# brudfors/UniRes

Measured on AMD Instinct MI355X. Metric: cg_iters_per_sec, higher is better.
Workload: dtype f32

## Files before the change

include/unires_hip.h:

```cpp
#ifndef UNIRES_HIP_H
#define UNIRES_HIP_H

#include <stdint.h>

#ifdef __cplusplus
extern "C" {
#endif

#define UNIRES_HIP_ABI_VERSION 1
#define UNIRES_MAX_TAPS 32

enum unires_status {
  UNIRES_OK = 0,
  UNIRES_ERR_NULL = 1,
  UNIRES_ERR_DIM = 2,
  UNIRES_ERR_ARG = 3,
  UNIRES_ERR_HIP = 4,
  UNIRES_ERR_ALLOC = 5,
  UNIRES_ERR_UNSUPPORTED = 6
};

enum unires_operator { UNIRES_OP_A = 0, UNIRES_OP_AT = 1, UNIRES_OP_ATA = 2 };

enum unires_regime {
// ... 48 lines not shown

int unires_div_fwd_zero(const float *src3, const int32_t dim[3], const float vx[3], float *dst,
                        void *stream);

int unires_dtd(const float *src, const int32_t dim[3], const float vx[3], float a, float c,
               float *dst, void *stream);


typedef struct unires_repeat {
  int32_t dim_x[3];
  int32_t dim_g[3];
  float M[12];
  int32_t ratio[3];
  int32_t ntaps[3];
  const float *taps[3];
  float scl;
  int32_t dim_thick;
  float tau;
} unires_repeat_t;

typedef struct unires_plan unires_plan_t;

int unires_plan_create(unires_plan_t **plan, const int32_t dim_y[3], const float vx_y[3],
                       int32_t regime, int32_t n_repeats, const unires_repeat_t *repeats,
                       float fov_tol);
int unires_plan_destroy(unires_plan_t *plan);
int unires_plan_set_repeat(unires_plan_t *plan, int32_t n, const unires_repeat_t *repeat);
int unires_plan_set_concurrency(unires_plan_t *plan, int32_t n_concurrent);
int64_t unires_plan_workspace_bytes(const unires_plan_t *plan);
int unires_plan_repeat_info(const unires_plan_t *plan, int32_t n, int32_t info[8]);
int unires_orient_of(const float M[12], int32_t perm[3], int32_t flip[3]);
int unires_plan_time_matvecs(unires_plan_t *plan, int32_t on);
int unires_plan_matvec_time(unires_plan_t *plan, int32_t *launches, double *total_us);

int unires_proj_apply(unires_plan_t *plan, int32_t n, int32_t op, const float *in, float *out,
                      void *stream);

int unires_ata_matvec(unires_plan_t *plan, float rho, float lam, const float *p, float *q,
                      double *dot_dev, void *stream);

int unires_rhs_assemble(unires_plan_t *plan, const float *const *x_ptrs, const float *w_c,
                        const float *z_c, float rho, float lam, float *b, void *stream);

int unires_atx_assemble(unires_plan_t *plan, const float *const *x_ptrs, float *atx,
                        void *stream);

int unires_rhs_from_atx(unires_plan_t *plan, const float *atx, const float *w_c,
                        const float *z_c, float rho, float lam, float *b, void *stream);

int unires_precond_build(unires_plan_t *plan, int32_t precond_mode, float rho, float lam,
                         float *m_out, void *stream);

int unires_precond_apply(unires_plan_t *plan, const float *in, float *out, void *stream);

int unires_cg_solve(unires_plan_t *plan, float rho, float lam, const float *b, float *x,
                    int32_t max_iter, double tol, int32_t stop_mode, int32_t precond_mode,
                    int32_t *iters_out, double *obj_trace, void *stream);

int unires_cg_solve_many(int32_t n, unires_plan_t *const *plans, const float *rho, const float *lam,
                         const float *const *b, float *const *x, int32_t max_iter, double tol,
                         int32_t stop_mode, int32_t precond_mode, int32_t *iters_out,
                         double *obj_trace, void *const *streams);


int unires_zw_update(const float *const *y_ptrs, const float *lam, int32_t n_channels,
                     const int32_t dim[3], const float vx[3], float rho, float alpha, float *z,
// ... 27 lines not shown
```

unires_amd/_lib.py:

```python
import ctypes as C
import os

_HERE = os.path.dirname(os.path.abspath(__file__))
LIB_PATH = os.environ.get('UNIRES_LIB') or os.path.join(_HERE, 'libunires_hip.so')

UNIRES_MAX_TAPS = 32
OP = {'A': 0, 'At': 1, 'AtA': 2}
REGIME_IDENTITY, REGIME_DENOISE, REGIME_SUPERRES = 0, 1, 2
STOP = {'e': 0, 'max_gain': 3, 'max_gain_guarded': 3, 'max_gain_fresh': 1, 'max_gain_recurred': 2}
PRECOND = {'none': 0, 'identity': 0, 'jacobi': 1, 'fft': 2}

c_i32x3 = C.c_int32 * 3
c_f32x3 = C.c_float * 3
c_f32x12 = C.c_float * 12
c_fptrx3 = C.POINTER(C.c_float) * 3


class Repeat(C.Structure):
    _fields_ = [('dim_x', c_i32x3), ('dim_g', c_i32x3), ('M', c_f32x12), ('ratio', c_i32x3),
                ('ntaps', c_i32x3), ('taps', c_fptrx3), ('scl', C.c_float),
                ('dim_thick', C.c_int32), ('tau', C.c_float)]


SIGNATURES = {
    'unires_last_error': (C.c_char_p, []),
    'unires_abi_version': (C.c_int, []),
    'unires_pull3d_affine': (C.c_int, [C.c_void_p, c_i32x3, c_f32x12, C.c_void_p, c_i32x3,
                                       C.c_float, C.c_void_p]),
    'unires_warp_label': (C.c_int, [C.c_void_p, c_i32x3, c_f32x12, C.c_void_p, c_i32x3,
                                    C.c_float, C.c_void_p]),
    'unires_pull3d_nearest': (C.c_int, [C.c_void_p, c_i32x3, c_f32x12, C.c_void_p, c_i32x3,
                                        C.c_float, C.c_void_p]),
    'unires_pull_grad3d_affine': (C.c_int, [C.c_void_p, c_i32x3, c_f32x12, C.c_void_p, c_i32x3,
                                            C.c_float, C.c_void_p]),
    'unires_push3d_affine': (C.c_int, [C.c_void_p, c_i32x3, c_f32x12, C.c_void_p, c_i32x3,
                                       C.c_float, C.c_float, C.c_int, C.c_void_p]),
    'unires_conv_down3d': (C.c_int, [C.c_void_p, c_i32x3, c_fptrx3, c_i32x3, c_i32x3, C.c_void_p,
                                     c_i32x3, C.c_float, C.c_int32, C.c_void_p]),
    'unires_conv_up3d': (C.c_int, [C.c_void_p, c_i32x3, c_fptrx3, c_i32x3, c_i32x3, C.c_void_p,
                                   c_i32x3, C.c_float, C.c_int32, C.c_void_p]),
    'unires_grad_fwd_zero': (C.c_int, [C.c_void_p, c_i32x3, c_f32x3, C.c_void_p, C.c_void_p]),
    'unires_div_fwd_zero': (C.c_int, [C.c_void_p, c_i32x3, c_f32x3, C.c_void_p, C.c_void_p]),
    'unires_dtd': (C.c_int, [C.c_void_p, c_i32x3, c_f32x3, C.c_float, C.c_float, C.c_void_p,
                             C.c_void_p]),
    'unires_plan_create': (C.c_int, [C.POINTER(C.c_void_p), c_i32x3, c_f32x3, C.c_int32,
                                     C.c_int32, C.POINTER(Repeat), C.c_float]),
    'unires_plan_destroy': (C.c_int, [C.c_void_p]),
    'unires_plan_set_repeat': (C.c_int, [C.c_void_p, C.c_int32, C.POINTER(Repeat)]),
    'unires_plan_set_concurrency': (C.c_int, [C.c_void_p, C.c_int32]),
    'unires_plan_workspace_bytes': (C.c_int64, [C.c_void_p]),
    'unires_orient_of': (C.c_int, [c_f32x12, c_i32x3, c_i32x3]),
    'unires_plan_repeat_info': (C.c_int, [C.c_void_p, C.c_int32, C.c_int32 * 8]),
    'unires_plan_time_matvecs': (C.c_int, [C.c_void_p, C.c_int32]),
    'unires_plan_matvec_time': (C.c_int, [C.c_void_p, C.POINTER(C.c_int32), C.POINTER(C.c_double)]),
    'unires_proj_apply': (C.c_int, [C.c_void_p, C.c_int32, C.c_int32, C.c_void_p, C.c_void_p,
                                    C.c_void_p]),
    'unires_ata_matvec': (C.c_int, [C.c_void_p, C.c_float, C.c_float, C.c_void_p, C.c_void_p,
                                    C.c_void_p, C.c_void_p]),
    'unires_rhs_assemble': (C.c_int, [C.c_void_p, C.POINTER(C.c_void_p), C.c_void_p, C.c_void_p,
                                      C.c_float, C.c_float, C.c_void_p, C.c_void_p]),
    'unires_atx_assemble': (C.c_int, [C.c_void_p, C.POINTER(C.c_void_p), C.c_void_p, C.c_void_p]),
    'unires_rhs_from_atx': (C.c_int, [C.c_void_p, C.c_void_p, C.c_void_p, C.c_void_p, C.c_float,
                                      C.c_float, C.c_void_p, C.c_void_p]),
    'unires_precond_build': (C.c_int, [C.c_void_p, C.c_int32, C.c_float, C.c_float, C.c_void_p,
                                       C.c_void_p]),
    'unires_precond_apply': (C.c_int, [C.c_void_p, C.c_void_p, C.c_void_p, C.c_void_p]),
    'unires_cg_solve': (C.c_int, [C.c_void_p, C.c_float, C.c_float, C.c_void_p, C.c_void_p,
                                  C.c_int32, C.c_double, C.c_int32, C.c_int32,
                                  C.POINTER(C.c_int32), C.POINTER(C.c_double), C.c_void_p]),
    'unires_cg_solve_many': (C.c_int, [C.c_int32, C.POINTER(C.c_void_p), C.POINTER(C.c_float),
                                       C.POINTER(C.c_float), C.POINTER(C.c_void_p), C.POINTER(C.c_void_p),
                                       C.c_int32, C.c_double, C.c_int32, C.c_int32, C.POINTER(C.c_int32),
                                       C.POINTER(C.c_double), C.POINTER(C.c_void_p)]),
    'unires_zw_update': (C.c_int, [C.POINTER(C.c_void_p), C.POINTER(C.c_float), C.c_int32, c_i32x3,
                                   c_f32x3, C.c_float, C.c_float, C.c_void_p, C.c_void_p,
                                   C.c_void_p, C.c_void_p]),
    'unires_nll_prior': (C.c_int, [C.POINTER(C.c_void_p), C.POINTER(C.c_float), C.c_int32, c_i32x3,
                                   c_f32x3, C.c_void_p, C.c_void_p]),
    'unires_scaling_sums': (C.c_int, [C.c_void_p, C.c_void_p, c_i32x3, C.c_int32, C.c_void_p,
                                      C.c_void_p]),
    'unires_rigid_sums': (C.c_int, [C.c_void_p, C.c_void_p, C.c_void_p, c_i32x3, C.c_float * 72,
                                    C.c_void_p, C.c_void_p]),
    'unires_clean_fov': (C.c_int, [C.c_void_p, c_i32x3, c_f32x12, c_i32x3, C.c_void_p]),
    'unires_masked_sse': (C.c_int, [C.c_void_p, C.c_void_p, C.c_int64, C.c_void_p, C.c_void_p]),
    'unires_mark_create': (C.c_int, [C.POINTER(C.c_void_p)]),
    'unires_mark_destroy': (C.c_int, [C.c_void_p]),
    'unires_mark_signal': (C.c_int, [C.c_void_p, C.c_uint64, C.c_void_p]),
# ... 45 lines not shown
```

unires_amd/_plan.py:

```python
import ctypes as C

import numpy as np
import torch

from . import _lib
from ._lib import (REGIME_DENOISE, REGIME_IDENTITY, REGIME_SUPERRES, Repeat, check, f3, i3)
from ._ops import FOV_TOL, _ptr, _stream, _vol, on_device
from .spatial import _m12, voxel_size


def proj_matrix(po, method):
    if method == 'super-resolution':
        return torch.linalg.solve(po.mat_y, po.rigid.mm(po.mat_yx)), tuple(po.dim_yx)
    if method == 'denoising':
        return torch.linalg.solve(po.mat_y, po.rigid.mm(po.mat_x)), tuple(po.dim_x)
    raise ValueError('Undefined method')


def regime_of(method, do_proj):
    if method not in ('denoising', 'super-resolution'):
        raise ValueError('Undefined method')
    if not do_proj:
        return REGIME_IDENTITY
    return REGIME_SUPERRES if method == 'super-resolution' else REGIME_DENOISE
# ... 50 lines not shown
    def rhs_buffer(self, like):
        buf = getattr(self, '_rhs_buf', None)
        if buf is None or buf.shape != like.shape or buf.device != like.device:
            buf = torch.empty_like(like)
            self._rhs_buf = buf
        return buf

    def close(self):
        if getattr(self, '_h', None) is not None and self._h:
            try:
                with torch.cuda.device(self.device):
                    self.lib.unires_plan_destroy(self._h)
            except Exception:
                self.lib.unires_plan_destroy(self._h)
            self._h = None

    __del__ = close

    @property
    def workspace_bytes(self):
        return int(self.lib.unires_plan_workspace_bytes(self._h))

    def repeat_info(self, n):
        info = (C.c_int32 * 8)()
        check(self.lib.unires_plan_repeat_info(self._h, int(n), info))
        v = list(info)
        return dict(perm=tuple(v[:3]), flip=tuple((v[3] >> j) & 1 for j in range(3)), pull2=bool(v[4]),
                    splat2_axis=None if v[5] == 0 else v[5] - 2, shift=bool(v[6] & 1), separable=bool(v[7]),
                    fused=bool(v[6] & 2))

    @on_device
    def time_matvecs(self, on=True):
        check(self.lib.unires_plan_time_matvecs(self._h, 2 if on == 2 else (1 if on else 0)))

    @on_device
    def matvec_time(self):
        n, us = C.c_int32(0), C.c_double(0.0)
        check(self.lib.unires_plan_matvec_time(self._h, C.byref(n), C.byref(us)))
        return int(n.value), float(us.value)

    @on_device
    def set_repeat(self, n, po, tau):
        keep = []
        r = _repeat_desc(po, tau, self.method, self.regime, keep)
        check(self.lib.unires_plan_set_repeat(self._h, n, C.byref(r)))

    def set_concurrency(self, n):
        n = max(1, int(n))
        if n != self._concurrency:
            check(self.lib.unires_plan_set_concurrency(self._h, n))
            self._concurrency = n

    def _y(self, t, name):
        v, _ = _vol(t, name)
        if tuple(v.shape) != self.dim_y:
            raise ValueError('unires_amd: %s has shape %s, expected %s'
                             % (name, tuple(v.shape), self.dim_y))
        return v

    @on_device
    def proj_apply(self, n, operator, dat):
        if operator not in _lib.OP:
            raise ValueError('Undefined operator')
        d, lead = _vol(dat)
        out_dim = self.dims_x[n] if operator == 'A' else self.dim_y
        in_dim = self.dims_x[n] if operator == 'At' else self.dim_y
# ... 137 lines not shown
```

unires_amd/csrc/api.hip:

```cpp
#include <math.h>
#include <stdio.h>
#include <stdlib.h>
#include <string.h>

#include <time.h>

#include <functional>
#include <map>
#include <mutex>
#include <new>
#include <string>
#include <vector>

#include "admm.hpp"
#include "aligned.hpp"
#include "cg.hpp"
#include "fftpre.hpp"
#include "fused.hpp"
#include "ops.hpp"
#include "orient.hpp"
#include "pull2.hpp"
#include "shift.hpp"
#include "splat2.hpp"
#include "ata1.hpp"
// ... 268 lines not shown
  int ctab_n = 0, ctab_cap = 0;
  unsigned ctab_step = 1, src_stride = 1;
  float *xytab_dev[2] = {nullptr, nullptr};
  int xytab_cap[2] = {0, 0};
  PullPlan pplan;
  ShiftPlan shift;
  F1Sched f1;
};

struct unires_plan {
  Dim3i dy;
  float vx[3];
  int regime;
  float fov_tol;
  std::vector<Repeat> reps;
  char *ws = nullptr;
  size_t ws_bytes = 0;
  float *r = nullptr, *p = nullptr, *ap = nullptr, *ax = nullptr;
  bool timing = false;
  bool twice = false;
  std::vector<std::pair<hipEvent_t, hipEvent_t>> tev;
  float *gbuf = nullptr;
  float *gbuf2 = nullptr;
  float *xbuf = nullptr;
  float *xperm = nullptr;
  double *part0 = nullptr, *part1 = nullptr;
  CgState *state = nullptr;
  size_t cap_g = 0, cap_x = 0;
  struct CgKey {
    const float *b = nullptr;
    float *x = nullptr;
    float rho = 0.f, lam = 0.f;
    int max_iter = -1, stop = -1, pre = -1;
    double tol = -1.0;
    bool operator==(const CgKey &o) const {
      return b == o.b && x == o.x && rho == o.rho && lam == o.lam && max_iter == o.max_iter &&
             stop == o.stop && pre == o.pre && tol == o.tol;
    }
  } cg_key;
  hipGraphExec_t cg_exec = nullptr;
  CgKey cg_chunk_key;
  hipGraphExec_t cg_start_exec = nullptr, cg_chunk_exec = nullptr;
  unsigned long long *progress = nullptr, *progress_dev = nullptr;
  unsigned cg_gen = 0;
  float *precM = nullptr;
  FftPre fft;
  float prec_rho = 0.f, prec_lam = 0.f;
  int prec_mode = UNIRES_PRECOND_IDENTITY;
  bool prec_ready = false;
  hipEvent_t last_use = nullptr;
  std::vector<hipStream_t> use_streams;
  bool captured_use = false;
  int concurrency = 1;
  int cap_s2 = 0, cap_f1 = 0;
};

static void drop_timing(unires_plan *pl) {
  for (auto &e : pl->tev) (void)hipEventDestroy(e.first), (void)hipEventDestroy(e.second);
  pl->tev.clear();
}

static void mark_use(unires_plan *pl, hipStream_t st) {
  hipStreamCaptureStatus cs = hipStreamCaptureStatusNone;
  if (hipStreamIsCapturing(st, &cs) != hipSuccess) {
    (void)hipGetLastError();
    cs = hipStreamCaptureStatusNone;
  }
  if (cs != hipStreamCaptureStatusNone) {
    pl->captured_use = true;
    return;
  }
  for (hipStream_t s : pl->use_streams)
    if (s == st) return;
  if (pl->use_streams.size() >= 8)
    pl->captured_use = true;
  else
    pl->use_streams.push_back(st);
}
// ... 337 lines not shown
  pl->ax = (float *)(pl->ws + o_ax);
  pl->gbuf = (float *)(pl->ws + o_g);
  pl->xbuf = (float *)(pl->ws + o_x);
  pl->xperm = (float *)(pl->ws + o_xp);
  pl->gbuf2 = need_sep ? (float *)(pl->ws + o_g2) : nullptr;
  pl->part0 = (double *)(pl->ws + o_p0);
  pl->part1 = (double *)(pl->ws + o_p1);
  pl->state = (CgState *)(pl->ws + o_st);
  e = hipMemset(pl->state, 0, sizeof(CgState));
  if (e != hipSuccess) {
    g_err = std::string("hipMemset: ") + hipGetErrorString(e);
    (void)hipFree(pl->ws);
    delete pl;
    return UNIRES_ERR_HIP;
  }
  for (Repeat &R : pl->reps) {
    int rc = UNIRES_OK;
    if (!rc) rc = build_repeat_kernels(pl, R);
    if (rc) {
      for (Repeat &Q : pl->reps) free_sched(Q);
      (void)hipFree(pl->ws);
      delete pl;
      return rc;
    }
  }
  *plan = pl;
  return UNIRES_OK;
}

extern "C" int unires_plan_destroy(unires_plan_t *plan) {
  if (!plan) return UNIRES_OK;
  if (plan->ws) (void)hipFree(plan->ws);
  if (plan->precM) (void)hipFree(plan->precM);
  if (plan->cg_exec) (void)hipGraphExecDestroy(plan->cg_exec);
  if (plan->cg_start_exec) (void)hipGraphExecDestroy(plan->cg_start_exec);
  if (plan->cg_chunk_exec) (void)hipGraphExecDestroy(plan->cg_chunk_exec);
  if (plan->progress) (void)hipHostFree(plan->progress);
  if (plan->last_use) (void)hipEventDestroy(plan->last_use);
  drop_timing(plan);
  fftpre_destroy(plan->fft);
  for (Repeat &R : plan->reps) free_sched(R);
  delete plan;
  return UNIRES_OK;
}

extern "C" int unires_plan_time_matvecs(unires_plan_t *plan, int32_t on) {
  if (!plan) return fail(UNIRES_ERR_NULL, "null argument");
  const bool twice = on == 2;
  if (twice != plan->twice) drop_cg_graph(plan);
  plan->twice = twice;
  plan->timing = on == 1;
  if (!plan->timing) drop_timing(plan);
  return UNIRES_OK;
}

extern "C" int unires_plan_matvec_time(unires_plan_t *plan, int32_t *launches, double *total_us) {
  if (!plan || !launches || !total_us) return fail(UNIRES_ERR_NULL, "null argument");
  *launches = 0, *total_us = 0.0;
  for (auto &e : plan->tev) {
    float ms = 0.f;
    HIP_TRY(hipEventSynchronize(e.second));
    HIP_TRY(hipEventElapsedTime(&ms, e.first, e.second));
    *total_us += 1e3 * (double)ms;
    ++*launches;
  }
  drop_timing(plan);
  return UNIRES_OK;
}

extern "C" int unires_plan_set_repeat(unires_plan_t *plan, int32_t n,
                                      const unires_repeat_t *repeat) {
  if (!plan || !repeat) return fail(UNIRES_ERR_NULL, "null argument");
  if (n < 0 || n >= (int)plan->reps.size()) return fail(UNIRES_ERR_ARG, "repeat index");
  Repeat tmp;
  int rc = fill_repeat(plan, repeat, tmp);
  if (rc) return rc;
  if (plan->regime != UNIRES_REGIME_IDENTITY &&
      (tmp.dim_g.numel() > plan->cap_g || tmp.dim_x.numel() > plan->cap_x))
    return fail(UNIRES_ERR_DIM, "new repeat exceeds the plan's workspace");
  if (plan->regime == UNIRES_REGIME_SUPERRES && (tmp.sep || tmp.hyb) && !plan->gbuf2)
    return fail(UNIRES_ERR_DIM, "new repeat needs the separable-conv scratch the plan was built without");
  await_use(plan);
  drop_cg_graph(plan);
  plan->prec_ready = false;
  {
// ... 476 lines not shown
  return UNIRES_OK;
}

extern "C" int unires_rhs_from_atx(unires_plan_t *plan, const float *atx, const float *w_c,
                                   const float *z_c, float rho, float lam, float *b,
                                   void *stream) {
  if (!plan || !atx || !w_c || !z_c || !b) return fail(UNIRES_ERR_NULL, "null argument");
  launch_div(w_c, z_c, 1.f, -rho, plan->dy, plan->vx, -lam, atx, b, (hipStream_t)stream);
  CHECK_LAUNCH();
  return UNIRES_OK;
}

static int cg_enqueue_start(unires_plan *pl, float rho, float lam, const float *b, float *x, double tol,
                            int stop_mode, const float *M, bool fft, unsigned long long *hostw,
                            hipStream_t st) {
  const size_t ny = pl->dy.numel();
  const bool check = tol != 0.0;
  CgState *S = pl->state;
  const int gv = vec_num_blocks(ny);
  HIP_TRY(hipMemsetAsync(&S->done, 0, sizeof(int), st));
  matvec(pl, rho, lam, x, pl->ap, nullptr, nullptr, st);
  const bool want_obj0 = check && stop_mode != UNIRES_STOP_RESIDUAL;
  launch_residual_init(b, pl->ap, x, pl->r, pl->p, ny, pl->part0, want_obj0 ? pl->part1 : nullptr,
                       M, st);
  if (fft) {
    if (fftpre_apply(pl->fft, pl->r, pl->fft.z, st)) return fail(UNIRES_ERR_HIP, "hipFFT execution failed");
    HIP_TRY(hipMemcpyAsync(pl->p, pl->fft.z, ny * sizeof(float), hipMemcpyDeviceToDevice, st));
    launch_dot(pl->r, pl->fft.z, ny, pl->part0, nullptr, st);
  }
  launch_sc_init(S, pl->part0, pl->part1, gv, stop_mode, check ? 1 : 0, hostw, st);
  return UNIRES_OK;
}

static int cg_enqueue_iters(unires_plan *pl, float rho, float lam, const float *b, float *x, int k_first,
                            int count, double tol, int stop_mode, const float *M, bool fft, bool dev_k,
                            unsigned long long *hostw, hipStream_t st) {
  const size_t ny = pl->dy.numel();
  const bool check = tol != 0.0;
  CgState *S = pl->state;
  const int *done = &S->done;
  const int gv = vec_num_blocks(ny);
  static const bool fold_on = getenv("UNIRES_CG_FOLD") && getenv("UNIRES_CG_FOLD")[0] == '1';
  const int gf = vec_num_blocks_fold(ny);
  for (int k = k_first; k < k_first + count; ++k) {
    const int kk = dev_k ? -1 : k;
    hipEvent_t ev0 = nullptr, ev1 = nullptr;
    if (pl->timing && hipEventCreate(&ev0) == hipSuccess) {
      if (hipEventCreate(&ev1) == hipSuccess) {
        (void)hipEventRecord(ev0, st);
      } else {
        (void)hipEventDestroy(ev0);
        ev0 = nullptr;
      }
    }
    if (pl->twice) (void)matvec(pl, rho, lam, pl->p, pl->ap, pl->part0, done, st);
    const int g = matvec(pl, rho, lam, pl->p, pl->ap, pl->part0, done, st);
    if (ev0 && ev1) {
      (void)hipEventRecord(ev1, st);
      if (pl->tev.size() >= 65536) {
        (void)hipEventDestroy(pl->tev.front().first), (void)hipEventDestroy(pl->tev.front().second);
        pl->tev.erase(pl->tev.begin());
      }
      pl->tev.emplace_back(ev0, ev1);
    }
    const bool guarded = check && stop_mode == UNIRES_STOP_MAXGAIN_GUARDED;
    const bool recur = check && (stop_mode == UNIRES_STOP_MAXGAIN_RECURRED || guarded);
    int obj_kind = 0;
    if (check && stop_mode == UNIRES_STOP_RESIDUAL) obj_kind = 1;
    if (recur) obj_kind = 2;
    const bool lazy_x = obj_kind == 0;
    if (fold_on && lazy_x && !fft && !dev_k) {
      launch_update_r_fold(S, pl->part0, g, k, pl->ap, pl->r, ny, pl->part1, M, st);
      launch_update_px_fold(S, pl->part1, gf, k, pl->r, pl->p, x, ny, M, st);
    } else {
      launch_sc_alpha(S, pl->part0, g, st);
      launch_update_xr(S, pl->p, pl->ap, lazy_x ? nullptr : x, pl->r, b, ny, pl->part0,
                       recur ? pl->part1 : nullptr, M, st);
      if (fft) {
        if (fftpre_apply(pl->fft, pl->r, pl->fft.z, st)) return fail(UNIRES_ERR_HIP, "hipFFT execution failed");
        launch_dot(pl->r, pl->fft.z, ny, pl->part0, done, st);
      }
      if (guarded)
        launch_sc_beta_guarded(S, pl->part0, pl->part1, gv, kk, tol, hostw, st);
      else
        launch_sc_beta(S, pl->part0, pl->part1, gv, kk, obj_kind, tol, obj_kind ? hostw : nullptr, st);
      launch_update_p(S, fft ? pl->fft.z : pl->r, pl->p, ny, M, lazy_x ? x : nullptr, st);
    }
    if (check && stop_mode == UNIRES_STOP_MAXGAIN) {
      const int go = matvec(pl, rho, lam, x, pl->ax, pl->part1, done, st, b);
      launch_sc_obj(S, pl->part1, go, kk, tol, hostw, st);
    }
    if (guarded) {
      const int go = matvec(pl, rho, lam, x, pl->ax, pl->part1, &S->skip_fresh, st, b);
      launch_sc_obj_guarded(S, pl->part1, go, kk, tol, hostw, st);
    }
  }
  return UNIRES_OK;
}

static int cg_enqueue(unires_plan *pl, float rho, float lam, const float *b, float *x, int max_iter,
                      double tol, int stop_mode, const float *M, bool fft, hipStream_t st) {
  const int rc = cg_enqueue_start(pl, rho, lam, b, x, tol, stop_mode, M, fft, nullptr, st);
  if (rc) return rc;
  return cg_enqueue_iters(pl, rho, lam, b, x, 1, max_iter, tol, stop_mode, M, fft, false, nullptr, st);
}

struct CgRun {
  unires_plan *pl = nullptr;
  float rho = 0.f, lam = 0.f;
  const float *b = nullptr;
  float *x = nullptr;
  int max_iter = 0, stop = 0, chunk = 2;
  double tol = 0.0;
  const float *M = nullptr;
  bool fft = false;
  hipStream_t st = nullptr;
  int enqueued = 0;
  unsigned gen = 0;
  bool finished = false;
  bool use_graph = false;
};

static void cg_resync_gen(unires_plan *pl) {
  (void)hipDeviceSynchronize();
  (void)hipGetLastError();
  unsigned g = pl->cg_gen;
  if (pl->state && hipMemcpy(&g, &pl->state->gen, sizeof(g), hipMemcpyDeviceToHost) == hipSuccess) pl->cg_gen = g;
  (void)hipGetLastError();
}

static int cg_chunk_size() {
  static const int k = [] {
    const char *e = getenv("UNIRES_CG_CHUNK");
    const int v = e ? atoi(e) : 2;
    return v < 1 ? 1 : (v > 64 ? 64 : v);
  }();
  return k;
// ... 187 lines not shown
  R.use_graph = cg_graphs_on() && !R.fft && !pl->timing;
  return R;
}

static int cg_read_back(unires_plan *pl, int max_iter, double tol, int32_t *iters_out, double *obj_trace,
                        hipStream_t st) {
  CgState *S = pl->state;
  int it = 0;
  HIP_TRY(hipMemcpyAsync(&it, &S->iters, sizeof(int), hipMemcpyDeviceToHost, st));
  if (obj_trace && tol != 0.0)
    HIP_TRY(hipMemcpyAsync(obj_trace, S->obj, sizeof(double) * (size_t)(std::min(max_iter, kMaxCgIter) + 1),
                           hipMemcpyDeviceToHost, st));
  HIP_TRY(hipStreamSynchronize(st));
  *iters_out = it;
  return UNIRES_OK;
}

extern "C" int unires_cg_solve(unires_plan_t *plan, float rho, float lam, const float *b, float *x,
                               int32_t max_iter, double tol, int32_t stop_mode,
                               int32_t precond_mode, int32_t *iters_out, double *obj_trace,
                               void *stream) {
  int rc = cg_check_args(plan, rho, lam, b, x, max_iter, tol, stop_mode, precond_mode);
  if (rc) return rc;
  const float *M = precond_mode == UNIRES_PRECOND_JACOBI ? plan->precM : nullptr;
  const bool fft = precond_mode == UNIRES_PRECOND_FFT;
  hipStream_t st = (hipStream_t)stream;
  unires_plan *pl = plan;
  mark_use(pl, st);

  if (stream_capturing(st) && tol != 0.0 && max_iter > kMaxCgIter)
    return fail(UNIRES_ERR_ARG, "a solve with a tolerance and more than 4096 iterations cannot join a stream capture "
                                "(it is fed to the device chunk by chunk, following its progress)");
  if (cg_chunked(tol, max_iter) && !(stream_capturing(st) && max_iter <= kMaxCgIter)) {
    std::vector<CgRun> runs(1, cg_make_run(pl, rho, lam, b, x, max_iter, tol, stop_mode, precond_mode, st));
    if ((rc = cg_run_start(runs[0]))) return rc;
    if ((rc = cg_runs_drive(runs))) return rc;
    mark_use(pl, st);
    CHECK_LAUNCH();
    return iters_out ? cg_read_back(pl, max_iter, tol, iters_out, obj_trace, st) : UNIRES_OK;
  }
  ++pl->cg_gen;

  unires_plan::CgKey key;
  key.b = b, key.x = x, key.rho = rho, key.lam = lam, key.max_iter = max_iter, key.stop = stop_mode;
  key.pre = precond_mode, key.tol = tol;
  const bool graphable = cg_graphs_on() && !fft && max_iter > 0 && !pl->timing;
  if (graphable && pl->cg_exec && pl->cg_key == key) {
    HIP_TRY(hipGraphLaunch(pl->cg_exec, st));
  } else {
    if (graphable && pl->cg_exec) drop_cg_graph(pl);
    rc = graphable ? capture_graph(st, &pl->cg_exec, [&] {
      return cg_enqueue(pl, rho, lam, b, x, max_iter, tol, stop_mode, M, fft, st);
    }) : -1;
    if (rc > 0) {
      cg_resync_gen(pl);
      return rc;
    }
    if (rc == 0) {
      pl->cg_key = key;
      if (hipGraphLaunch(pl->cg_exec, st) != hipSuccess) {
        cg_resync_gen(pl);
        return fail(UNIRES_ERR_HIP, "hipGraphLaunch failed");
      }
    } else if ((rc = cg_enqueue(pl, rho, lam, b, x, max_iter, tol, stop_mode, M, fft, st))) {
      cg_resync_gen(pl);
      return rc;
    }
  }
  mark_use(pl, st);
  CHECK_LAUNCH();
  return iters_out ? cg_read_back(pl, max_iter, tol, iters_out, obj_trace, st) : UNIRES_OK;
}

extern "C" int unires_cg_solve_many(int32_t n, unires_plan_t *const *plans, const float *rho, const float *lam,
                                    const float *const *b, float *const *x, int32_t max_iter, double tol,
                                    int32_t stop_mode, int32_t precond_mode, int32_t *iters_out,
                                    double *obj_trace, void *const *streams) {
  if (n < 1 || !plans || !rho || !lam || !b || !x || !streams) return fail(UNIRES_ERR_NULL, "null argument");
  for (int c = 0; c < n; ++c) {
    const int rc = cg_check_args(plans[c], rho[c], lam[c], b[c], x[c], max_iter, tol, stop_mode, precond_mode);
    if (rc) return rc;
    for (int d = 0; d < c; ++d)
      if (plans[d] == plans[c]) return fail(UNIRES_ERR_ARG, "one plan per solve");
  }
  bool capturing = false;
  for (int c = 0; c < n; ++c) capturing = capturing || stream_capturing((hipStream_t)streams[c]);
  if (capturing && tol != 0.0 && max_iter > kMaxCgIter)
    return fail(UNIRES_ERR_ARG, "a solve with a tolerance and more than 4096 iterations cannot join a stream capture "
                                "(it is fed to the device chunk by chunk, following its progress)");
  for (int c = 0; c < n; ++c) mark_use(plans[c], (hipStream_t)streams[c]);
  if (!cg_chunked(tol, max_iter) || (capturing && max_iter <= kMaxCgIter)) {
    for (int c = 0; c < n; ++c) {
      const int rc = unires_cg_solve(plans[c], rho[c], lam[c], b[c], x[c], max_iter, tol, stop_mode, precond_mode,
                                     nullptr, nullptr, streams[c]);
      if (rc) return rc;
    }
  } else {
    std::vector<CgRun> runs;
    for (int c = 0; c < n; ++c)
      runs.push_back(cg_make_run(plans[c], rho[c], lam[c], b[c], x[c], max_iter, tol, stop_mode, precond_mode,
                                 (hipStream_t)streams[c]));
    for (CgRun &R : runs) {
      const int rc = cg_run_start(R);
      if (rc) return rc;
    }
    const int rc = cg_runs_drive(runs);
    if (rc) return rc;
    for (int c = 0; c < n; ++c) mark_use(plans[c], (hipStream_t)streams[c]);
    CHECK_LAUNCH();
  }
  if (iters_out)
    for (int c = 0; c < n; ++c) {
      const int rc = cg_read_back(plans[c], max_iter, tol, iters_out + c,
                                  obj_trace ? obj_trace + (size_t)c * (std::min(max_iter, kMaxCgIter) + 1) : nullptr,
                                  (hipStream_t)streams[c]);
      if (rc) return rc;
    }
  return UNIRES_OK;
}

static int check_channels(const float *const *y_ptrs, const float *lam, int32_t n) {
  if (!y_ptrs || !lam) return fail(UNIRES_ERR_NULL, "null argument");
  if (n < 1 || n > 4096) return fail(UNIRES_ERR_ARG, "channel count out of range");
  for (int c = 0; c < n; ++c)
    if (!y_ptrs[c]) return fail(UNIRES_ERR_NULL, "null channel pointer");
  return UNIRES_OK;
}

static int reduce_scratch(hipStream_t st, size_t ndoubles, double **out) {
  static std::mutex mu;
  static std::map<std::pair<int, hipStream_t>, std::pair<double *, size_t>> scratch;
// ... 176 lines not shown
```

unires_amd/csrc/cg.hip:

```cpp
#include "cg.hpp"

namespace unires {

static inline int vec_blocks(size_t n) {
  size_t b = (n / 4 + kBlock - 1) / kBlock;
  if (b < 1) b = 1;
  const size_t cap = 4096;
  return (int)(b < cap ? b : cap);
}

#define GRID_STRIDE_VEC4(n)                                                   \
  const size_t n4 = (n) / 4;                                                  \
  const size_t stride = (size_t)gridDim.x * blockDim.x;                       \
  const size_t tid0 = (size_t)blockIdx.x * blockDim.x + threadIdx.x

__device__ __forceinline__ float4 ld4(const float *p, size_t i) {
  return reinterpret_cast<const float4 *>(p)[i];
}
__device__ __forceinline__ void st4(float *p, size_t i, float4 v) {
  reinterpret_cast<float4 *>(p)[i] = v;
}
typedef float f4v __attribute__((ext_vector_type(4)));
__device__ __forceinline__ float4 ld4_stream(const float *p, size_t i) {
#ifdef UNIRES_CG_X_PLAIN
// ... 134 lines not shown
    const double t2 = block_sum(ob);
    if (threadIdx.x == 0) part_obj[blockIdx.x] = t2;
  }
}

template <bool XUPD>
__global__ void __launch_bounds__(kBlock)
    k_update_p(const CgState *__restrict__ st, const float *__restrict__ r, float *__restrict__ p,
               size_t n, const float *__restrict__ M, float *__restrict__ x) {
  if (st->done) return;
  const float beta = (float)st->beta, alpha = (float)st->alpha;
  GRID_STRIDE_VEC4(n);
  for (size_t i = tid0; i < n4; i += stride) {
    const float4 vr = zval4(ld4(r, i), M, i);
    float4 vp = ld4(p, i);
    if (XUPD) {
      float4 vx = ld4_stream(x, i);
      vx.x = __fadd_rn(vx.x, __fmul_rn(alpha, vp.x));
      vx.y = __fadd_rn(vx.y, __fmul_rn(alpha, vp.y));
      vx.z = __fadd_rn(vx.z, __fmul_rn(alpha, vp.z));
      vx.w = __fadd_rn(vx.w, __fmul_rn(alpha, vp.w));
      st4_stream(x, i, vx);
    }
    vp.x = __fadd_rn(__fmul_rn(beta, vp.x), vr.x);
    vp.y = __fadd_rn(__fmul_rn(beta, vp.y), vr.y);
    vp.z = __fadd_rn(__fmul_rn(beta, vp.z), vr.z);
    vp.w = __fadd_rn(__fmul_rn(beta, vp.w), vr.w);
    st4(p, i, vp);
  }
  for (size_t i = n4 * 4 + tid0; i < n; i += stride) {
    const float vp = p[i];
    if (XUPD) x[i] = __fadd_rn(x[i], __fmul_rn(alpha, vp));
    p[i] = __fadd_rn(__fmul_rn(beta, vp), zval1(r[i], M, i));
  }
}

__global__ void __launch_bounds__(kBlock)
    k_axpy(float a, const float *__restrict__ x, float *__restrict__ y, size_t n) {
  const size_t stride = (size_t)gridDim.x * blockDim.x;
  for (size_t i = (size_t)blockIdx.x * blockDim.x + threadIdx.x; i < n; i += stride)
    y[i] = fmaf(a, x[i], y[i]);
}

__device__ __forceinline__ double reduce_all(const double *__restrict__ part, int g) {
  __shared__ double s_tot[kBlock / kWave];
  double v = 0.0;
  int i = threadIdx.x;
  for (; i + 7 * kBlock < g; i += 8 * kBlock) {
    double t[8];
#pragma unroll
    for (int u = 0; u < 8; ++u) t[u] = part[i + u * kBlock];
#pragma unroll
    for (int u = 0; u < 8; ++u) v += t[u];
  }
  for (; i < g; i += kBlock) v += part[i];
  v = wave_sum(v);
  __syncthreads();
  if ((threadIdx.x & (kWave - 1)) == 0) s_tot[threadIdx.x / kWave] = v;
  __syncthreads();
  double tot = 0.0;
#pragma unroll
  for (int w = 0; w < kBlock / kWave; ++w) tot += s_tot[w];
  return tot;
}

constexpr int kFoldIt = 4;
// ... 295 lines not shown
void launch_update_px_fold(CgState *s, const double *part_rr, int g, int k, const float *r, float *p,
                           float *x, size_t n, const float *M, hipStream_t st) {
  hipLaunchKernelGGL(k_update_px_fold, dim3(vec_blocks_fold(n)), dim3(kBlock), 0, st, s, part_rr, g, k, r, p,
                     x, n, M);
}

void launch_residual_init(const float *b, const float *ax, const float *x, float *r, float *p,
                          size_t n, double *part_rr, double *part_obj, const float *M,
                          hipStream_t st) {
  hipLaunchKernelGGL(k_residual_init, dim3(vec_blocks(n)), dim3(kBlock), 0, st, b, ax, x, r, p, n,
                     part_rr, part_obj, M);
}
void launch_dot(const float *a, const float *b, size_t n, double *part, const int *done,
                hipStream_t st) {
  hipLaunchKernelGGL(k_dot, dim3(vec_blocks(n)), dim3(kBlock), 0, st, a, b, n, part, done);
}
void launch_update_xr(const CgState *s, const float *p, const float *ap, float *x, float *r,
                      const float *b, size_t n, double *part_rr, double *part_obj,
                      const float *M, hipStream_t st) {
  if (x)
    hipLaunchKernelGGL(k_update_xr<true>, dim3(vec_blocks(n)), dim3(kBlock), 0, st, s, p, ap, x, r, b,
                       n, part_rr, part_obj, M);
  else
    hipLaunchKernelGGL(k_update_xr<false>, dim3(vec_blocks(n)), dim3(kBlock), 0, st, s, p, ap, x, r,
                       b, n, part_rr, part_obj, M);
}
void launch_update_p(const CgState *s, const float *r, float *p, size_t n, const float *M, float *x,
                     hipStream_t st) {
  if (x)
    hipLaunchKernelGGL(k_update_p<true>, dim3(vec_blocks(n)), dim3(kBlock), 0, st, s, r, p, n, M, x);
  else
    hipLaunchKernelGGL(k_update_p<false>, dim3(vec_blocks(n)), dim3(kBlock), 0, st, s, r, p, n, M, x);
}
__global__ void __launch_bounds__(kBlock) k_scale_shift(float a, float c, float *__restrict__ y, size_t n) {
  const size_t stride = (size_t)gridDim.x * blockDim.x;
  for (size_t i = (size_t)blockIdx.x * blockDim.x + threadIdx.x; i < n; i += stride)
    y[i] = __fadd_rn(__fmul_rn(a, y[i]), c);
}
void launch_scale_shift(float a, float c, float *y, size_t n, hipStream_t st) {
  hipLaunchKernelGGL(k_scale_shift, dim3(vec_blocks(n) * 4 > 4096 ? 4096 : vec_blocks(n) * 4),
                     dim3(kBlock), 0, st, a, c, y, n);
}
__global__ void __launch_bounds__(kBlock) k_fill(float v, float *__restrict__ y, size_t n) {
  const size_t stride = (size_t)gridDim.x * blockDim.x;
  for (size_t i = (size_t)blockIdx.x * blockDim.x + threadIdx.x; i < n; i += stride) y[i] = v;
}
void launch_fill(float v, float *y, size_t n, hipStream_t st) {
  hipLaunchKernelGGL(k_fill, dim3(vec_blocks(n) * 4 > 4096 ? 4096 : vec_blocks(n) * 4), dim3(kBlock), 0,
                     st, v, y, n);
}
__global__ void __launch_bounds__(kBlock)
    k_divide(const float *__restrict__ a, const float *__restrict__ m, float *__restrict__ y, size_t n) {
  const size_t stride = (size_t)gridDim.x * blockDim.x;
  for (size_t i = (size_t)blockIdx.x * blockDim.x + threadIdx.x; i < n; i += stride)
    y[i] = __fdiv_rn(a[i], m[i]);
}
void launch_div(const float *a, const float *m, float *y, size_t n, hipStream_t st) {
  hipLaunchKernelGGL(k_divide, dim3(vec_blocks(n) * 4 > 4096 ? 4096 : vec_blocks(n) * 4), dim3(kBlock), 0,
                     st, a, m, y, n);
}
void launch_axpy(float a, const float *x, float *y, size_t n, hipStream_t st) {
  hipLaunchKernelGGL(k_axpy, dim3(vec_blocks(n) * 4 > 4096 ? 4096 : vec_blocks(n) * 4),
                     dim3(kBlock), 0, st, a, x, y, n);
}
void launch_sc_init(CgState *s, const double *part_rr, const double *part_obj, int g, int mode,
                    int check, unsigned long long *hostw, hipStream_t st) {
// ... 29 lines not shown
```

unires_amd/csrc/cg.hpp:

```cpp
#pragma once
#include "common.hpp"

namespace unires {

constexpr int kMaxCgIter = 4096;

struct CgState {
  double rz, pAp, alpha, beta, obj_max, obj_min;
  int done, iters;
  unsigned gen, pad_;
  double rzpp[2];
  double obj[kMaxCgIter + 1];
  int skip_fresh;
  int fresh_prev_ok;
  double rec_prev, fresh_prev, gain_rec;
};

__host__ __device__ inline unsigned long long cg_progress_word(unsigned gen, int done, int iters) {
  return ((unsigned long long)gen << 32) | (done ? 0x80000000ull : 0ull) | (unsigned)(iters & 0x7fffffff);
}

int vec_num_blocks(size_t n);
void launch_residual_init(const float *b, const float *ax, const float *x, float *r, float *p,
                          size_t n, double *part_rr, double *part_obj, const float *M,
                          hipStream_t st);
void launch_dot(const float *a, const float *b, size_t n, double *part, const int *done,
                hipStream_t st);
void launch_update_xr(const CgState *s, const float *p, const float *ap, float *x, float *r,
                      const float *b, size_t n, double *part_rr, double *part_obj, const float *M,
                      hipStream_t st);
void launch_update_p(const CgState *s, const float *r, float *p, size_t n, const float *M, float *x,
                     hipStream_t st);
void launch_scale_shift(float a, float c, float *y, size_t n, hipStream_t st);
void launch_fill(float v, float *y, size_t n, hipStream_t st);
void launch_div(const float *a, const float *m, float *y, size_t n, hipStream_t st);
void launch_axpy(float a, const float *x, float *y, size_t n, hipStream_t st);
void launch_sc_init(CgState *s, const double *part_rr, const double *part_obj, int g, int mode,
                    int check, unsigned long long *hostw, hipStream_t st);
void launch_sc_alpha(CgState *s, const double *part, int g, hipStream_t st);
void launch_sc_beta(CgState *s, const double *part_rr, const double *part_obj, int g, int k,
                    int obj_kind, double tol, unsigned long long *hostw, hipStream_t st);
void launch_sc_obj(CgState *s, const double *part, int g, int k, double tol, unsigned long long *hostw,
                   hipStream_t st);
void launch_sc_beta_guarded(CgState *s, const double *part_rr, const double *part_obj, int g, int k, double tol,
                            unsigned long long *hostw, hipStream_t st);
void launch_sc_obj_guarded(CgState *s, const double *part, int g, int k, double tol, unsigned long long *hostw,
                           hipStream_t st);
void launch_sum_to(const double *part, int g, double *out, hipStream_t st);
int vec_num_blocks_fold(size_t n);
void launch_update_r_fold(CgState *s, const double *part_pap, int g, int k, const float *ap, float *r,
                          size_t n, double *part_rr, const float *M, hipStream_t st);
void launch_update_px_fold(CgState *s, const double *part_rr, int g, int k, const float *r, float *p,
                           float *x, size_t n, const float *M, hipStream_t st);

}
```

Before: 4852.

## Defer CG iterate updates via a ring of search directions flushed in batches

```diff
diff --git a/include/unires_hip.h b/include/unires_hip.h
--- a/include/unires_hip.h
+++ b/include/unires_hip.h
@@ -104,6 +104,7 @@
 int unires_orient_of(const float M[12], int32_t perm[3], int32_t flip[3]);
 int unires_plan_time_matvecs(unires_plan_t *plan, int32_t on);
 int unires_plan_matvec_time(unires_plan_t *plan, int32_t *launches, double *total_us);
+int unires_plan_cg_ring(unires_plan_t *plan, int32_t k, int32_t *last);
 
 int unires_proj_apply(unires_plan_t *plan, int32_t n, int32_t op, const float *in, float *out,
                       void *stream);
diff --git a/unires_amd/_lib.py b/unires_amd/_lib.py
--- a/unires_amd/_lib.py
+++ b/unires_amd/_lib.py
@@ -53,6 +53,7 @@
     'unires_plan_repeat_info': (C.c_int, [C.c_void_p, C.c_int32, C.c_int32 * 8]),
     'unires_plan_time_matvecs': (C.c_int, [C.c_void_p, C.c_int32]),
     'unires_plan_matvec_time': (C.c_int, [C.c_void_p, C.POINTER(C.c_int32), C.POINTER(C.c_double)]),
+    'unires_plan_cg_ring': (C.c_int, [C.c_void_p, C.c_int32, C.POINTER(C.c_int32)]),
     'unires_proj_apply': (C.c_int, [C.c_void_p, C.c_int32, C.c_int32, C.c_void_p, C.c_void_p,
                                     C.c_void_p]),
     'unires_ata_matvec': (C.c_int, [C.c_void_p, C.c_float, C.c_float, C.c_void_p, C.c_void_p,
diff --git a/unires_amd/_plan.py b/unires_amd/_plan.py
--- a/unires_amd/_plan.py
+++ b/unires_amd/_plan.py
@@ -106,6 +106,11 @@
     @on_device
     def time_matvecs(self, on=True):
         check(self.lib.unires_plan_time_matvecs(self._h, 2 if on == 2 else (1 if on else 0)))
+
+    def cg_ring(self, k=0):
+        last = C.c_int32(0)
+        check(self.lib.unires_plan_cg_ring(self._h, int(k), C.byref(last)))
+        return int(last.value)
 
     @on_device
     def matvec_time(self):
diff --git a/unires_amd/csrc/api.hip b/unires_amd/csrc/api.hip
--- a/unires_amd/csrc/api.hip
+++ b/unires_amd/csrc/api.hip
@@ -324,10 +324,11 @@
     float *x = nullptr;
     float rho = 0.f, lam = 0.f;
     int max_iter = -1, stop = -1, pre = -1;
+    int ring = 1;
     double tol = -1.0;
     bool operator==(const CgKey &o) const {
       return b == o.b && x == o.x && rho == o.rho && lam == o.lam && max_iter == o.max_iter &&
-             stop == o.stop && pre == o.pre && tol == o.tol;
+             stop == o.stop && pre == o.pre && ring == o.ring && tol == o.tol;
     }
   } cg_key;
   hipGraphExec_t cg_exec = nullptr;
@@ -336,6 +337,11 @@
   unsigned long long *progress = nullptr, *progress_dev = nullptr;
   unsigned cg_gen = 0;
   float *precM = nullptr;
+  float *ring = nullptr;
+  int ring_slots = 0;
+  bool ring_tried = false;
+  int ring_req = 0;
+  int last_ring = 1;
   FftPre fft;
   float prec_rho = 0.f, prec_lam = 0.f;
   int prec_mode = UNIRES_PRECOND_IDENTITY;
@@ -739,6 +745,7 @@
   if (!plan) return UNIRES_OK;
   if (plan->ws) (void)hipFree(plan->ws);
   if (plan->precM) (void)hipFree(plan->precM);
+  if (plan->ring) (void)hipFree(plan->ring);
   if (plan->cg_exec) (void)hipGraphExecDestroy(plan->cg_exec);
   if (plan->cg_start_exec) (void)hipGraphExecDestroy(plan->cg_start_exec);
   if (plan->cg_chunk_exec) (void)hipGraphExecDestroy(plan->cg_chunk_exec);
@@ -758,6 +765,18 @@
   plan->twice = twice;
   plan->timing = on == 1;
   if (!plan->timing) drop_timing(plan);
+  return UNIRES_OK;
+}
+
+extern "C" int unires_plan_cg_ring(unires_plan_t *plan, int32_t k, int32_t *last) {
+  if (!plan) return fail(UNIRES_ERR_NULL, "null argument");
+  if (k < 0) return fail(UNIRES_ERR_ARG, "ring size must be >= 0");
+  if (k > 0) {
+    const int v = std::min<int>(k, kMaxRing);
+    if (v != plan->ring_req) drop_cg_graph(plan);
+    plan->ring_req = v;
+  }
+  if (last) *last = plan->last_ring;
   return UNIRES_OK;
 }
 
@@ -1300,18 +1319,33 @@
   return UNIRES_OK;
 }
 
+static bool cg_fold_on() {
+  static const bool on = getenv("UNIRES_CG_FOLD") && getenv("UNIRES_CG_FOLD")[0] == '1';
+  return on;
+}
+
+static float *ring_slot(unires_plan *pl, int j) {
+  return j == 0 ? pl->p : pl->ring + (size_t)(j - 1) * (align_up(pl->dy.numel() * 4) / 4);
+}
+
 static int cg_enqueue_iters(unires_plan *pl, float rho, float lam, const float *b, float *x, int k_first,
                             int count, double tol, int stop_mode, const float *M, bool fft, bool dev_k,
-                            unsigned long long *hostw, hipStream_t st) {
+                            unsigned long long *hostw, hipStream_t st, int ring = 1) {
   const size_t ny = pl->dy.numel();
   const bool check = tol != 0.0;
   CgState *S = pl->state;
   const int *done = &S->done;
   const int gv = vec_num_blocks(ny);
-  static const bool fold_on = getenv("UNIRES_CG_FOLD") && getenv("UNIRES_CG_FOLD")[0] == '1';
+  const bool fold_on = cg_fold_on();
   const int gf = vec_num_blocks_fold(ny);
+  if (ring > 1 && (check || fft || dev_k || fold_on || ring > kMaxRing || ring - 1 > pl->ring_slots))
+    return fail(UNIRES_ERR_ARG, "deferred iterate update outside its scope");
+  RingPtrs rp = {};
+  for (int j = 0; j < ring && ring > 1; ++j) rp.p[j] = ring_slot(pl, j);
   for (int k = k_first; k < k_first + count; ++k) {
     const int kk = dev_k ? -1 : k;
+    const int slot = ring > 1 ? (k - k_first) % ring : 0;
+    float *p = ring > 1 ? ring_slot(pl, slot) : pl->p;
     hipEvent_t ev0 = nullptr, ev1 = nullptr;
     if (pl->timing && hipEventCreate(&ev0) == hipSuccess) {
       if (hipEventCreate(&ev1) == hipSuccess) {
@@ -1321,8 +1355,8 @@
         ev0 = nullptr;
       }
     }
-    if (pl->twice) (void)matvec(pl, rho, lam, pl->p, pl->ap, pl->part0, done, st);
-    const int g = matvec(pl, rho, lam, pl->p, pl->ap, pl->part0, done, st);
+    if (pl->twice) (void)matvec(pl, rho, lam, p, pl->ap, pl->part0, done, st);
+    const int g = matvec(pl, rho, lam, p, pl->ap, pl->part0, done, st);
     if (ev0 && ev1) {
       (void)hipEventRecord(ev1, st);
       if (pl->tev.size() >= 65536) {
@@ -1342,7 +1376,7 @@
       launch_update_px_fold(S, pl->part1, gf, k, pl->r, pl->p, x, ny, M, st);
     } else {
       launch_sc_alpha(S, pl->part0, g, st);
-      launch_update_xr(S, pl->p, pl->ap, lazy_x ? nullptr : x, pl->r, b, ny, pl->part0,
+      launch_update_xr(S, p, pl->ap, lazy_x ? nullptr : x, pl->r, b, ny, pl->part0,
                        recur ? pl->part1 : nullptr, M, st);
       if (fft) {
         if (fftpre_apply(pl->fft, pl->r, pl->fft.z, st)) return fail(UNIRES_ERR_HIP, "hipFFT execution failed");
@@ -1352,7 +1386,12 @@
         launch_sc_beta_guarded(S, pl->part0, pl->part1, gv, kk, tol, hostw, st);
       else
         launch_sc_beta(S, pl->part0, pl->part1, gv, kk, obj_kind, tol, obj_kind ? hostw : nullptr, st);
-      launch_update_p(S, fft ? pl->fft.z : pl->r, pl->p, ny, M, lazy_x ? x : nullptr, st);
+      if (ring > 1 && (slot == ring - 1 || k == k_first + count - 1))
+        launch_update_p_flush(S, pl->r, rp, slot + 1, ring_slot(pl, (slot + 1) % ring), ny, M, x, st);
+      else if (ring > 1)
+        launch_update_p_ring(S, pl->r, p, ring_slot(pl, slot + 1), slot, ny, M, st);
+      else
+        launch_update_p(S, fft ? pl->fft.z : pl->r, pl->p, ny, M, lazy_x ? x : nullptr, st);
     }
     if (check && stop_mode == UNIRES_STOP_MAXGAIN) {
       const int go = matvec(pl, rho, lam, x, pl->ax, pl->part1, done, st, b);
@@ -1367,10 +1406,43 @@
 }
 
 static int cg_enqueue(unires_plan *pl, float rho, float lam, const float *b, float *x, int max_iter,
-                      double tol, int stop_mode, const float *M, bool fft, hipStream_t st) {
+                      double tol, int stop_mode, const float *M, bool fft, hipStream_t st, int ring) {
   const int rc = cg_enqueue_start(pl, rho, lam, b, x, tol, stop_mode, M, fft, nullptr, st);
   if (rc) return rc;
-  return cg_enqueue_iters(pl, rho, lam, b, x, 1, max_iter, tol, stop_mode, M, fft, false, nullptr, st);
+  return cg_enqueue_iters(pl, rho, lam, b, x, 1, max_iter, tol, stop_mode, M, fft, false, nullptr, st, ring);
+}
+
+static bool stream_capturing(hipStream_t st);
+static int cg_ring_prepare(unires_plan *pl, hipStream_t st) {
+  static const int env_k = [] {
+    const char *e = getenv("UNIRES_CG_RING");
+    return e ? atoi(e) : 8;
+  }();
+  int want = pl->ring_req > 0 ? pl->ring_req : env_k;
+  want = std::max(1, std::min(want, kMaxRing));
+  if (want <= 1) return 1;
+  if (!pl->ring_tried) {
+    if (stream_capturing(st)) return 1;
+    pl->ring_tried = true;
+    const size_t slot = align_up(pl->dy.numel() * 4);
+    size_t budget = 0;
+    if (const char *e = getenv("UNIRES_CG_RING_MB")) {
+      budget = (size_t)std::max(0.0, atof(e) * 1048576.0);
+    } else {
+      size_t free_b = 0, total_b = 0;
+      if (hipMemGetInfo(&free_b, &total_b) == hipSuccess) budget = free_b / 8;
+      (void)hipGetLastError();
+    }
+    const int n = (int)std::min<size_t>((size_t)(want - 1), budget / slot);
+    if (n < 1) return 1;
+    if (hipMalloc((void **)&pl->ring, (size_t)n * slot) != hipSuccess) {
+      (void)hipGetLastError();
+      pl->ring = nullptr;
+      return 1;
+    }
+    pl->ring_slots = n;
+  }
+  return std::min(want, pl->ring_slots + 1);
 }
 
 struct CgRun {
@@ -1624,6 +1696,7 @@
     return fail(UNIRES_ERR_ARG, "a solve with a tolerance and more than 4096 iterations cannot join a stream capture "
                                 "(it is fed to the device chunk by chunk, following its progress)");
   if (cg_chunked(tol, max_iter) && !(stream_capturing(st) && max_iter <= kMaxCgIter)) {
+    pl->last_ring = 1;
     std::vector<CgRun> runs(1, cg_make_run(pl, rho, lam, b, x, max_iter, tol, stop_mode, precond_mode, st));
     if ((rc = cg_run_start(runs[0]))) return rc;
     if ((rc = cg_runs_drive(runs))) return rc;
@@ -1632,17 +1705,19 @@
     return iters_out ? cg_read_back(pl, max_iter, tol, iters_out, obj_trace, st) : UNIRES_OK;
   }
   ++pl->cg_gen;
+  const int ring = tol == 0.0 && !fft && !cg_fold_on() && max_iter > 0 ? cg_ring_prepare(pl, st) : 1;
+  pl->last_ring = ring;
 
   unires_plan::CgKey key;
   key.b = b, key.x = x, key.rho = rho, key.lam = lam, key.max_iter = max_iter, key.stop = stop_mode;
-  key.pre = precond_mode, key.tol = tol;
+  key.pre = precond_mode, key.tol = tol, key.ring = ring;
   const bool graphable = cg_graphs_on() && !fft && max_iter > 0 && !pl->timing;
   if (graphable && pl->cg_exec && pl->cg_key == key) {
     HIP_TRY(hipGraphLaunch(pl->cg_exec, st));
   } else {
     if (graphable && pl->cg_exec) drop_cg_graph(pl);
     rc = graphable ? capture_graph(st, &pl->cg_exec, [&] {
-      return cg_enqueue(pl, rho, lam, b, x, max_iter, tol, stop_mode, M, fft, st);
+      return cg_enqueue(pl, rho, lam, b, x, max_iter, tol, stop_mode, M, fft, st, ring);
     }) : -1;
     if (rc > 0) {
       cg_resync_gen(pl);
@@ -1654,7 +1729,7 @@
         cg_resync_gen(pl);
         return fail(UNIRES_ERR_HIP, "hipGraphLaunch failed");
       }
-    } else if ((rc = cg_enqueue(pl, rho, lam, b, x, max_iter, tol, stop_mode, M, fft, st))) {
+    } else if ((rc = cg_enqueue(pl, rho, lam, b, x, max_iter, tol, stop_mode, M, fft, st, ring))) {
       cg_resync_gen(pl);
       return rc;
     }
@@ -1689,6 +1764,7 @@
     }
   } else {
     std::vector<CgRun> runs;
+    for (int c = 0; c < n; ++c) plans[c]->last_ring = 1;
     for (int c = 0; c < n; ++c)
       runs.push_back(cg_make_run(plans[c], rho[c], lam[c], b[c], x[c], max_iter, tol, stop_mode, precond_mode,
                                  (hipStream_t)streams[c]));
diff --git a/unires_amd/csrc/cg.hip b/unires_amd/csrc/cg.hip
--- a/unires_amd/csrc/cg.hip
+++ b/unires_amd/csrc/cg.hip
@@ -190,6 +190,85 @@
     const float vp = p[i];
     if (XUPD) x[i] = __fadd_rn(x[i], __fmul_rn(alpha, vp));
     p[i] = __fadd_rn(__fmul_rn(beta, vp), zval1(r[i], M, i));
+  }
+}
+
+
+__global__ void __launch_bounds__(kBlock)
+    k_update_p_ring(CgState *__restrict__ st, const float *__restrict__ r, const float *__restrict__ p_in,
+                    float *__restrict__ p_out, int slot, size_t n, const float *__restrict__ M) {
+  const int done = st->done;
+  if (blockIdx.x == 0 && threadIdx.x == 0) st->ahist[slot] = st->alpha, st->committed[slot] = done ? 0 : 1;
+  if (done) return;
+  const float beta = (float)st->beta;
+  GRID_STRIDE_VEC4(n);
+  for (size_t i = tid0; i < n4; i += stride) {
+    const float4 vz = zval4(ld4(r, i), M, i);
+    float4 vp = ld4_stream(p_in, i);
+    vp.x = __fadd_rn(__fmul_rn(beta, vp.x), vz.x);
+    vp.y = __fadd_rn(__fmul_rn(beta, vp.y), vz.y);
+    vp.z = __fadd_rn(__fmul_rn(beta, vp.z), vz.z);
+    vp.w = __fadd_rn(__fmul_rn(beta, vp.w), vz.w);
+    st4(p_out, i, vp);
+  }
+  for (size_t i = n4 * 4 + tid0; i < n; i += stride)
+    p_out[i] = __fadd_rn(__fmul_rn(beta, p_in[i]), zval1(r[i], M, i));
+}
+
+__global__ void __launch_bounds__(kBlock)
+    k_update_p_flush(CgState *__restrict__ st, const float *__restrict__ r, RingPtrs ring, int m, float *p_out,
+                     size_t n, const float *__restrict__ M, float *__restrict__ x) {
+  const int done = st->done;
+  const float beta = (float)st->beta;
+  float a[kMaxRing];
+  bool c[kMaxRing];
+  bool any = false;
+#pragma unroll
+  for (int j = 0; j < kMaxRing; ++j) {
+    c[j] = false, a[j] = 0.f;
+    if (j < m - 1) c[j] = st->committed[j] != 0, a[j] = (float)st->ahist[j];
+    if (j == m - 1) c[j] = !done, a[j] = (float)st->alpha;
+    any = any || c[j];
+  }
+  if (!any) return;
+  GRID_STRIDE_VEC4(n);
+  for (size_t i = tid0; i < n4; i += stride) {
+    float4 vz = make_float4(0.f, 0.f, 0.f, 0.f);
+    if (!done) vz = zval4(ld4(r, i), M, i);
+    float4 vx = ld4_stream(x, i);
+    float4 vp[kMaxRing];
+#pragma unroll
+    for (int j = 0; j < kMaxRing; ++j)
+      if (c[j]) vp[j] = ld4_stream(ring.p[j], i);
+#pragma unroll
+    for (int j = 0; j < kMaxRing; ++j) {
+      if (!c[j]) continue;
+      vx.x = __fadd_rn(vx.x, __fmul_rn(a[j], vp[j].x));
+      vx.y = __fadd_rn(vx.y, __fmul_rn(a[j], vp[j].y));
+      vx.z = __fadd_rn(vx.z, __fmul_rn(a[j], vp[j].z));
+      vx.w = __fadd_rn(vx.w, __fmul_rn(a[j], vp[j].w));
+      if (j == m - 1) {
+        float4 b = vp[j];
+        b.x = __fadd_rn(__fmul_rn(beta, b.x), vz.x);
+        b.y = __fadd_rn(__fmul_rn(beta, b.y), vz.y);
+        b.z = __fadd_rn(__fmul_rn(beta, b.z), vz.z);
+        b.w = __fadd_rn(__fmul_rn(beta, b.w), vz.w);
+        st4(p_out, i, b);
+      }
+    }
+    st4_stream(x, i, vx);
+  }
+  for (size_t i = n4 * 4 + tid0; i < n; i += stride) {
+    float vx = x[i], own = 0.f;
+#pragma unroll
+    for (int j = 0; j < kMaxRing; ++j) {
+      if (!c[j]) continue;
+      const float pj = ring.p[j][i];
+      vx = __fadd_rn(vx, __fmul_rn(a[j], pj));
+      if (j == m - 1) own = pj;
+    }
+    x[i] = vx;
+    if (!done) p_out[i] = __fadd_rn(__fmul_rn(beta, own), zval1(r[i], M, i));
   }
 }
 
@@ -551,6 +630,14 @@
   else
     hipLaunchKernelGGL(k_update_p<false>, dim3(vec_blocks(n)), dim3(kBlock), 0, st, s, r, p, n, M, x);
 }
+void launch_update_p_ring(CgState *s, const float *r, const float *p_in, float *p_out, int slot, size_t n,
+                          const float *M, hipStream_t st) {
+  hipLaunchKernelGGL(k_update_p_ring, dim3(vec_blocks(n)), dim3(kBlock), 0, st, s, r, p_in, p_out, slot, n, M);
+}
+void launch_update_p_flush(CgState *s, const float *r, const RingPtrs &ring, int m, float *p_out, size_t n,
+                           const float *M, float *x, hipStream_t st) {
+  hipLaunchKernelGGL(k_update_p_flush, dim3(vec_blocks(n)), dim3(kBlock), 0, st, s, r, ring, m, p_out, n, M, x);
+}
 __global__ void __launch_bounds__(kBlock) k_scale_shift(float a, float c, float *__restrict__ y, size_t n) {
   const size_t stride = (size_t)gridDim.x * blockDim.x;
   for (size_t i = (size_t)blockIdx.x * blockDim.x + threadIdx.x; i < n; i += stride)
diff --git a/unires_amd/csrc/cg.hpp b/unires_amd/csrc/cg.hpp
--- a/unires_amd/csrc/cg.hpp
+++ b/unires_amd/csrc/cg.hpp
@@ -4,6 +4,7 @@
 namespace unires {
 
 constexpr int kMaxCgIter = 4096;
+constexpr int kMaxRing = 8;
 
 struct CgState {
   double rz, pAp, alpha, beta, obj_max, obj_min;
@@ -14,6 +15,11 @@
   int skip_fresh;
   int fresh_prev_ok;
   double rec_prev, fresh_prev, gain_rec;
+  double ahist[kMaxRing];
+  int committed[kMaxRing];
+};
+struct RingPtrs {
+  const float *p[kMaxRing];
 };
 
 __host__ __device__ inline unsigned long long cg_progress_word(unsigned gen, int done, int iters) {
@@ -31,6 +37,10 @@
                       hipStream_t st);
 void launch_update_p(const CgState *s, const float *r, float *p, size_t n, const float *M, float *x,
                      hipStream_t st);
+void launch_update_p_ring(CgState *s, const float *r, const float *p_in, float *p_out, int slot, size_t n,
+                          const float *M, hipStream_t st);
+void launch_update_p_flush(CgState *s, const float *r, const RingPtrs &ring, int m, float *p_out, size_t n,
+                           const float *M, float *x, hipStream_t st);
 void launch_scale_shift(float a, float c, float *y, size_t n, hipStream_t st);
 void launch_fill(float v, float *y, size_t n, hipStream_t st);
 void launch_div(const float *a, const float *m, float *y, size_t n, hipStream_t st);
```

New measurement: 5127 (median of 6 runs). 5.7% higher.
